# Validation-m3sSAGE/GCN_Recommendation

Hardware: AMD Instinct MI355X
Metric: propagated edges/sec (SpMM) + Recall@20, Amazon-Books 3-layer d=64 (higher is better)
Workload: dtype f32; 1 GPU; C3 full Amazon-Books-2023 shape (10.3M users x 4.4M items x 29.5M interactions); generator=powerlaw, users=10300000, items=4400000, interactions=29500000, nnz=56305746, d=64, layers=3, brands=0, content_dim=0, hub_threshold=128, hub_mode=exact, emu_min_degree=1024, parallelism=single

## Files before the change

gcn_recommendation_amd/csrc/lgcn_engine.hip:

```cpp
#include "lgcn_kernels.h"

#include <string.h>
#include <algorithm>
#include <functional>
#include <new>
#include <vector>

namespace lgcn_detail {
int g_rows_per_group = 0;
int g_unroll = 0;
int g_mean_prefetch = 0;
int g_min_groups = 0;
int g_emu_margin = (128 << 4) | 4;
int g_sample_blocks = 0;
int g_fusion_bwd_blocks = 0;
}

namespace {
__global__ void k_coo_inspect(const int64_t* __restrict__ rows, const int64_t* __restrict__ cols,
                              int64_t nnz, int32_t n_rows, int32_t n_cols, int32_t* flags) {
    const int64_t j = (int64_t)blockIdx.x * blockDim.x + threadIdx.x;
    if (j >= nnz) return;
    const int64_t r = rows[j], c = cols[j];
    int f = 0;
// ... 356 lines not shown

int scale_rows(const lgcn_rows_t& x, int32_t n_rows, int32_t d, float div, float* y, int64_t ldy,
               hipStream_t s, bool sum = false) {
    const bool vec_ok = rows_aligned(x) && al16(y) && (ldy % 4 == 0);
    const Geo g = pick_geo(d, vec_ok);
    ScaleF f{&x, n_rows, g.dW, div, y, ldy, sum, s};
    return dispatch_geo(g, f);
}

struct MeanEmptyF {
    const int32_t* row_ids; int32_t n; const lgcn_rows_t* e0; int32_t dW; float div;
    int32_t inv_bits; float* y; int64_t ldy; hipStream_t s;
    template <typename V, int G, int NV> int operator()() const {
        return launch_mean_empty_t<V, G, NV>(row_ids, n, *e0, dW, div, inv_bits, y, ldy, s);
    }
};

int mean_empty(const int32_t* row_ids, int32_t n, const lgcn_epilogue_t& ep_in, float* y,
               int64_t ldy, int32_t d, hipStream_t s) {
    const lgcn_epilogue_t ep = with_pow2(ep_in);
    const bool vec_ok = rows_aligned(ep.prev0) && al16(y) && (ldy % 4 == 0);
    const Geo g = pick_geo(d, vec_ok);
    MeanEmptyF f{row_ids, n, &ep.prev0, g.dW, ep.div, ep.pad, y, ldy, s};
    return dispatch_geo(g, f);
}

lgcn_rows_t dense_rows(const float* p, int32_t n, int64_t ld) {
    lgcn_rows_t r;
    r.p0 = r.p1 = r.p2 = p;
    r.end0 = r.end1 = n;
    r.ld = ld;
    return r;
}

int valid_geom(int32_t n_rows, int32_t d) {
    if (n_rows < 0 || d < 1 || d > 2048) return LGCN_EINVAL;
    return 0;
}

}

template <typename V>
__global__ __launch_bounds__(256) void k_add_nonzero(const V* __restrict__ src, V* __restrict__ dst,
                                                     int64_t m) {
    for (int64_t i = (int64_t)blockIdx.x * 256 + threadIdx.x; i < m;
         i += (int64_t)gridDim.x * 256) {
// ... 914 lines not shown
        return LGCN_EINVAL;
    for (int i = 0; i < 2 * kSegs; ++i)
        if (int e = check_plan(plans + i)) return e;
    return 0;
}

bool classes_hold(const lgcn_sides_t& sd, const lgcn_hub_plan_t* plans) {
    for (int j = 0; j < 2; ++j) {
        const lgcn_hub_plan_t& p = plans[2 * 3 + j];
        if (p.emu_part_rows[0] > sd.part_rows[0] || p.emu_part_rows[1] > sd.part_rows[1])
            return false;
    }
    return true;
}

struct LayerIO {
    lgcn_rows_t x;
    float xdiv;
    const uint32_t* x_nz;
    float* y;
    lgcn_epilogue_t ep;
};

int seg_layer(const int32_t* rowptr, const lgcn_edge_t* edges, const int32_t* row_ids,
              int32_t lo, int32_t hi, const lgcn_hub_plan_t* plans, int k, int g,
              const LayerIO& io, int32_t d, const lgcn_sched* sc, const Lane& L, Deps* dp,
              int32_t empty_tail = 0) {
    if (empty_tail > 0) {
        hi -= empty_tail;
        if (io.ep.mode == LGCN_EPI_MEAN)
            if (int e = mean_empty(row_ids + hi, empty_tail, io.ep, io.y, d, d, L.main)) return e;
    }
    if (hi <= lo) {
        if (dp && dp->defer && sc)
            for (int i = 0; i < 2; ++i)
                if (int e = record(sc, L.main, &dp->part_done[i])) return e;
        return 0;
    }
    const int h = (k - 1) * kSegs + g;
    lgcn_sched v;
    const lgcn_sched* vp = nullptr;
    if (L.view) {
        v = *L.view;
        v.t0 = sc->timing_sides ? sc->timing_sides[2 * h] : nullptr;
        v.t1 = sc->timing_sides ? sc->timing_sides[2 * h + 1] : nullptr;
        v.trace = sc->trace_sides ? sc->trace_sides + h * 8 : nullptr;
        vp = &v;
    }
    Deps local;
    Deps* dq = dp;
    if (!vp && dp && dp->defer && sc) {
        local = *dp;
        local.defer = false;
        dq = &local;
    }
    if (int e = plan_layer(rowptr + lo, edges, row_ids + lo, hi - lo, plans[2 * g + (k & 1)],
                           io.x, io.xdiv, io.x_nz, io.y, d, d, io.ep, vp, L.main, dq))
        return e;
    if (dq == &local)
        for (int i = 0; i < 2; ++i)
            if (int e = record(sc, L.main, &dp->part_done[i])) return e;
    return 0;
}

int run_sides(const int32_t* rowptr, const lgcn_edge_t* edges, const int32_t* row_ids,
              const lgcn_sides_t& sd, const lgcn_hub_plan_t* plans, int32_t d, int32_t K,
              const std::function<LayerIO(int)>& layer, const lgcn_sched* sched, hipStream_t s,
              const int32_t* empty_tail = nullptr) {
    Lane lanes[2];
    bool l1_aux = false;
    if (sched) sched->pool->next = 0;
    const bool two = make_lanes(sched, s, lanes, l1_aux);
    const bool cap = capture_restricted(s);
    const bool classes = sched && sched->classes && classes_hold(sd, plans) && !cap;
    if (sched) sched->pool->state[3] = classes ? 1 : 0;
    const int32_t lo[kSegs] = {0, sd.class_end[0], sd.class_end[1], sd.split};
    const int32_t hi[kSegs] = {sd.class_end[0], sd.class_end[1], sd.split, 0};
    auto seg_hi = [&](int g, int32_t n) { return g == 3 ? n : hi[g]; };
    const int32_t n = sd.n;
    if (int e = fork_lanes(sched, two, lanes[1], s)) return e;
    constexpr int KM = LGCN_MAX_LAYERS + 2;
    hipEvent_t cls[KM][3] = {}, ab[KM] = {}, rest[KM] = {}, part[KM][2] = {};
    for (int k = 1; k <= K; ++k) {
        const LayerIO io = layer(k);
        const bool mean = io.ep.mode == LGCN_EPI_MEAN;
        {
            const Lane& L = lanes[(k + 1 + K) & 1];
            Deps dp;
            if (classes && k >= 2) {
                dp.part_wait[0] = cls[k - 1][0];
                dp.part_wait[1] = ab[k - 1];
            }
            dp.defer = k < K && sched && !cap;
            if (k == K && mean && sched && sched->lk_normal && two && l1_aux && !cap &&
                sched->n_aux >= 3)
                dp.lk = sched->aux[2];
            if (mean && k >= 2) {
                dp.late[0] = rest[k - 1];
                dp.late_emu[0] = part[k - 1][0];
                dp.late_emu[1] = part[k - 1][1];
            }
            if (int e = seg_layer(rowptr, edges, row_ids, sd.split, n, plans, k, 3, io, d, sched,
                                  L, &dp, empty_tail ? empty_tail[3] : 0))
                return e;
            if (k < K && sched) {
                if (int e = record(sched, L.main, &rest[k])) return e;
                part[k][0] = dp.part_done[0];
                part[k][1] = dp.part_done[1];
            }
        }
        {
            const Lane& L = lanes[(k + K) & 1];
            static const int up[3] = {0, 1, 2}, down[3] = {2, 1, 0};
            const int* order = k == 1 ? up : down;
            for (int t = 0; t < 3; ++t) {
                const int c = order[t];
                if (k >= 2 && (c <= 1 || !classes))
                    if (int e = wait_ev(L.main, part[k - 1][1])) return e;
                if (k >= 2 && (c == 0 || !classes))
                    if (int e = wait_ev(L.main, part[k - 1][0])) return e;
                Deps dp;
                if (mean && k >= 2) dp.late[0] = cls[k - 1][c];
                if (int e = seg_layer(rowptr, edges, row_ids, lo[c], seg_hi(c, n), plans, k, c,
                                      io, d, sched, L, &dp, empty_tail ? empty_tail[c] : 0))
                    return e;
                if (sched)
                    if (int e = record(sched, L.main, &cls[k][c])) return e;
            }
            ab[k] = k == 1 ? cls[k][1] : cls[k][0];
        }
    }
    return join_lanes(sched, two, lanes[1], s);
}
}

extern "C" {

int lgcn_sched_create(void* const* aux_streams, int32_t n_aux, lgcn_sched_t** out) {
    if (!out || n_aux < 1 || n_aux > 7 || !aux_streams) return LGCN_EINVAL;
    for (int i = 0; i < n_aux; ++i)
        if (!aux_streams[i]) return LGCN_EINVAL;
    lgcn_sched* sc = new (std::nothrow) lgcn_sched();
    EventPool* pool = new (std::nothrow) EventPool();
    if (!sc || !pool) {
        delete sc;
        delete pool;
        return LGCN_EINVAL;
// ... 171 lines not shown
int lgcn_propagate_forward_sides(const int32_t* rowptr, const lgcn_edge_t* edges,
                                 const int32_t* row_ids, const lgcn_sides_t* sides,
                                 const lgcn_hub_plan_t* plans, lgcn_rows_t emb, int32_t d,
                                 int32_t K, float* const* layer_bufs_host, float* out,
                                 const lgcn_sched_t* sched, void* stream) {
    return lgcn_propagate_forward_sides_lean(rowptr, edges, row_ids, sides, plans, nullptr, emb, d,
                                             K, layer_bufs_host, out, sched, stream);
}

int lgcn_propagate_forward_sides_lean(const int32_t* rowptr, const lgcn_edge_t* edges,
                                      const int32_t* row_ids, const lgcn_sides_t* sides,
                                      const lgcn_hub_plan_t* plans, const lgcn_lean_t* lean,
                                      lgcn_rows_t emb, int32_t d, int32_t K,
                                      float* const* layer_bufs_host, float* out,
                                      const lgcn_sched_t* sched, void* stream) {
    const int32_t n = sides ? sides->n : -1;
    if (int e = valid_geom(n, d)) return e;
    if (K < 0 || !out) return LGCN_EINVAL;
    if (K > LGCN_MAX_LAYERS) return LGCN_ETOOMANY;
    if (K > 1 && !layer_bufs_host) return LGCN_EINVAL;
    hipStream_t s = S(stream);
    if (K == 0) return scale_rows(emb, n, d, 1.0f, out, d, s, true);
    if (int e = check_sides(rowptr, row_ids, n, sides, plans)) return e;
    auto layer = [&](int k) {
        LayerIO io;
        memset(&io, 0, sizeof(io));
        io.x = (k == 1) ? emb : dense_rows(layer_bufs_host[k - 2], n, d);
        io.xdiv = 1.f;
        if (k < K) {
            io.ep.mode = LGCN_EPI_STORE;
            io.y = layer_bufs_host[k - 1];
        } else {
            io.ep.mode = LGCN_EPI_MEAN;
            io.ep.n_prev = K;
            io.ep.div = (float)(K + 1);
            io.ep.prev0 = emb;
            for (int i = 0; i + 1 < K; ++i) io.ep.prev_dense[i] = layer_bufs_host[i];
            io.ep.ld_prev = d;
            io.y = out;
        }
        return io;
    };
    if (lean) {
        const int32_t b[kSegs + 1] = {0, sides->class_end[0], sides->class_end[1], sides->split, n};
        for (int g = 0; g < kSegs; ++g)
            if (lean->empty_tail[g] < 0 || lean->empty_tail[g] > b[g + 1] - b[g])
                return LGCN_EINVAL;
    }
    return run_sides(rowptr, edges, row_ids, *sides, plans, d, K, layer, sched, s,
                     lean ? lean->empty_tail : nullptr);
}

int lgcn_propagate_backward_sides(const int32_t* rowptr, const lgcn_edge_t* edges,
                                  const int32_t* row_ids, const lgcn_sides_t* sides,
                                  const lgcn_hub_plan_t* plans, lgcn_rows_t grad_out,
                                  const uint32_t* grad_nz, int32_t d, int32_t K, float* work_h,
                                  float* grad_e0, const lgcn_sched_t* sched, void* stream) {
    const int32_t n = sides ? sides->n : -1;
    if (int e = valid_geom(n, d)) return e;
    if (K < 0 || !grad_out.p0 || !grad_e0) return LGCN_EINVAL;
    if (K > LGCN_MAX_LAYERS) return LGCN_ETOOMANY;
    hipStream_t s = S(stream);
    if (K == 0) return scale_rows(grad_out, n, d, 1.0f, grad_e0, d, s);
    if (K > 1 && !work_h) return LGCN_EINVAL;
    if (int e = check_sides(rowptr, row_ids, n, sides, plans)) return e;
    auto out_of = [&](int k) { return ((K - k) % 2 == 0) ? grad_e0 : work_h; };
    auto layer = [&](int k) {
        LayerIO io;
        memset(&io, 0, sizeof(io));
        io.x = k == 1 ? grad_out : dense_rows(out_of(k - 1), n, d);
        io.xdiv = k == 1 ? (float)(K + 1) : 1.f;
        io.x_nz = k == 1 ? grad_nz : nullptr;
        io.y = out_of(k);
// ... 46 lines not shown
```

gcn_recommendation_amd/csrc/lgcn_kernels.h:

```cpp
#pragma once
#include <hip/hip_runtime.h>
#include <hipcub/hipcub.hpp>

#include <stdint.h>
#include <string.h>

#include "lgcn.h"


namespace lgcn_detail {
extern int g_rows_per_group;
extern int g_unroll;
extern int g_mean_prefetch;
extern int g_min_groups;

struct LayerArgs {
    const int32_t* rowptr;
    const lgcn_edge_t* edges;
    const int32_t* row_ids;
    int32_t n_rows, thr;
    const lgcn_hub_item_t* items;
    int32_t n_items;
    float* partials;
    lgcn_rows_t x;
// ... 540 lines not shown
template <typename V, int G, int NV>
__global__ __launch_bounds__(kBlock) void k_mean_empty(const int32_t* __restrict__ row_ids,
                                                       int32_t n_rows, lgcn_rows_t e0, int32_t dW,
                                                       float div, int32_t inv_bits,
                                                       float* __restrict__ y, int64_t ldy) {
    using T = VT<V>;
    constexpr int RPB = kBlock / G;
    const int lane = threadIdx.x & (G - 1);
    const int64_t slot = (int64_t)blockIdx.x * RPB + threadIdx.x / G;
    if (slot >= n_rows) return;
    const int32_t row = row_ids[slot];
    const float* xr = seg_row(e0, row);
#pragma unroll
    for (int q = 0; q < NV; ++q) {
        const int c = lane + q * G;
        if (c < dW)
            store_out<V>(y + (int64_t)row * ldy + c * T::W,
                         div_exact<V>(T::add(load_stream<V>(xr + c * T::W), T::zero()), div,
                                      inv_bits));
    }
}

template <typename V, int G, int NV>
__global__ __launch_bounds__(kBlock) void k_rows_nonzero(lgcn_rows_t x, int32_t n_rows, int32_t dW,
                                                         uint32_t* __restrict__ mask,
                                                         int32_t* __restrict__ count) {
    using T = VT<V>;
    constexpr int RPB = kBlock / G;
    constexpr int ROWS = 256;
    __shared__ uint32_t words[ROWS / 32];
    const int lane = threadIdx.x & (G - 1);
    const int grp = threadIdx.x / G;
    if (threadIdx.x < ROWS / 32) words[threadIdx.x] = 0;
    __syncthreads();
    const int64_t base = (int64_t)blockIdx.x * ROWS;
    for (int i = grp; i < ROWS; i += RPB) {
        const int64_t r = base + i;
        bool nz = false;
        if (r < n_rows) {
            const float* xr = seg_row(x, (int32_t)r);
#pragma unroll
            for (int q = 0; q < NV; ++q) {
                const int c = lane + q * G;
                if (c < dW) {
                    const V v = T::load(xr + c * T::W);
                    if constexpr (T::W == 4) nz |= !(v.x == 0.f && v.y == 0.f && v.z == 0.f && v.w == 0.f);
// ... 166 lines not shown
template <typename V, int G, int NV>
int launch_scale_t(const lgcn_rows_t& x, int32_t n_rows, int32_t dW, float div, float* y,
                   int64_t ldy, bool sum, hipStream_t s) {
    constexpr int RPB = kBlock / G;
    const int64_t grid = ((int64_t)n_rows + RPB - 1) / RPB;
    if (grid == 0) return 0;
    if (sum)
        hipLaunchKernelGGL((k_scale_rows<V, G, NV, true>), dim3((uint32_t)grid), dim3(kBlock), 0,
                           s, x, n_rows, dW, div, y, ldy);
    else
        hipLaunchKernelGGL((k_scale_rows<V, G, NV>), dim3((uint32_t)grid), dim3(kBlock), 0, s, x,
                           n_rows, dW, div, y, ldy);
    return last_err();
}

template <typename V, int G, int NV>
int launch_mean_empty_t(const int32_t* row_ids, int32_t n_rows, const lgcn_rows_t& e0, int32_t dW,
                        float div, int32_t inv_bits, float* y, int64_t ldy, hipStream_t s) {
    constexpr int RPB = kBlock / G;
    const int64_t grid = ((int64_t)n_rows + RPB - 1) / RPB;
    if (grid == 0) return 0;
    hipLaunchKernelGGL((k_mean_empty<V, G, NV>), dim3((uint32_t)grid), dim3(kBlock), 0, s, row_ids,
                       n_rows, e0, dW, div, inv_bits, y, ldy);
    return last_err();
}

template <typename F>
int dispatch_geo(const Geo& g, const F& f) {
#define LGCN_CASE(VT_, G_, NV_) \
    if (g.G == G_ && g.NV == NV_) return f.template operator()<VT_, G_, NV_>();
    if (g.vec) {
        LGCN_CASE(float4, 4, 1)
        LGCN_CASE(float4, 8, 1)
        LGCN_CASE(float4, 16, 1)
        LGCN_CASE(float4, 32, 1)
        LGCN_CASE(float4, 64, 1)
        LGCN_CASE(float4, 64, 2)
        LGCN_CASE(float4, 64, 4)
        LGCN_CASE(float4, 64, 8)
    } else {
        LGCN_CASE(float, 4, 1)
        LGCN_CASE(float, 8, 1)
        LGCN_CASE(float, 16, 1)
        LGCN_CASE(float, 32, 1)
        LGCN_CASE(float, 64, 1)
        LGCN_CASE(float, 64, 2)
// ... 28 lines not shown
```

gcn_recommendation_amd/engine.py:

```python
import ctypes
import os
import threading

import numpy as np
import torch

_PKG = os.path.dirname(os.path.abspath(__file__))
LIB_PATH = os.path.join(_PKG, "liblgcn_engine.so")

LGCN_EPI_STORE, LGCN_EPI_MEAN, LGCN_EPI_ADD = 0, 1, 2
LGCN_SCATTER_STORE, LGCN_SCATTER_ADD = 0, 1
LGCN_MAX_LAYERS = 16
COO_ROWS_UNSORTED, COO_OUT_OF_RANGE, COO_COLS_UNSORTED = 1, 2, 4
INT32_MAX = 2 ** 31 - 1
TUNE_ROWS_PER_GROUP, TUNE_UNROLL, TUNE_MEAN_PREFETCH, TUNE_MIN_GROUPS = 1, 2, 3, 4
TUNE_EMU_MARGIN = 6
TUNE_SAMPLE_BLOCKS = 7
TUNE_FUSION_BWD_BLOCKS = 8
FUSION_BWD_CHUNK = 2048
SCHED_SLOTS0, SCHED_SLOTS1, SCHED_CHAIN, SCHED_TIMING_START, SCHED_TIMING_END, SCHED_TRACE = \
    1, 2, 3, 4, 5, 6
SCHED_TRACE_SIDES, SCHED_TIMING_SIDES = 7, 8
SCHED_CLASSES = 16
SCHED_LK_NORMAL = 17
# ... 60 lines not shown
                ("addend", RowsT), ("addend_nz", ctypes.c_void_p)]


class PlanT(ctypes.Structure):
    _fields_ = [("items", ctypes.c_void_p), ("rows", ctypes.c_void_p), ("partials", ctypes.c_void_p),
                ("emu_blocks", ctypes.c_void_p), ("emu_rows", ctypes.c_void_p),
                ("emu_rel", ctypes.c_void_p), ("emu_meta", ctypes.c_void_p),
                ("emu_stage", ctypes.c_void_p),
                ("threshold", ctypes.c_int32), ("n_items", ctypes.c_int32),
                ("n_rows", ctypes.c_int32), ("n_pre", ctypes.c_int32),
                ("n_emu_blocks", ctypes.c_int32), ("n_emu_rows", ctypes.c_int32),
                ("emu_part_rows", ctypes.c_int32 * 2), ("emu_part_blocks", ctypes.c_int32 * 2),
                ("emu_scratch_blocks", ctypes.c_int32), ("emu_live", ctypes.c_void_p),
                ("emu_part_max_blocks", ctypes.c_int32 * 2), ("emu_out", ctypes.c_void_p)]


class SidesT(ctypes.Structure):
    _fields_ = [("n", ctypes.c_int32), ("split", ctypes.c_int32), ("class_end", ctypes.c_int32 * 2),
                ("part_rows", ctypes.c_int32 * 2)]


class LeanT(ctypes.Structure):
    _fields_ = [("empty_tail", ctypes.c_int32 * 4)]


class AdamTensorT(ctypes.Structure):
    _fields_ = [("p", ctypes.c_void_p), ("g", ctypes.c_void_p), ("m", ctypes.c_void_p),
                ("v", ctypes.c_void_p), ("n", ctypes.c_int64), ("step_size", ctypes.c_double),
                ("bc2_sqrt", ctypes.c_double)]


class AdamHyperT(ctypes.Structure):
    _fields_ = [("lerp_w", ctypes.c_double), ("beta2", ctypes.c_double),
                ("one_minus_beta2", ctypes.c_double), ("eps", ctypes.c_double),
                ("weight_decay", ctypes.c_double)]


class LgcnError(RuntimeError):
    pass


_lib = None
_lib_lock = threading.Lock()

_P, _I32, _I64 = ctypes.c_void_p, ctypes.c_int32, ctypes.c_int64
ABI = [
# ... 75 lines not shown
    ("lgcn_live_scratch_bytes", ctypes.c_size_t, [_I32, _I32]),
    ("lgcn_live_rows", ctypes.c_int, [_P, _P, _I32, _P, _I32, RowsT, ctypes.c_float, _P, _P, _I64,
                                      _I32, ctypes.POINTER(EpilogueT), _I32, _I32, _P, _P]),
    ("lgcn_live_flags", ctypes.c_void_p, [_P, _I32, _I32]),
    ("lgcn_chain_rows", ctypes.c_int, [_P, _P, _P, _I32, RowsT, ctypes.c_float, _P, _I64, _I32,
                                       ctypes.POINTER(EpilogueT), _P]),
    ("lgcn_sched_create", ctypes.c_int, [_P, _I32, ctypes.POINTER(ctypes.c_void_p)]),
    ("lgcn_sched_destroy", ctypes.c_int, [_P]),
    ("lgcn_sched_set", ctypes.c_int, [_P, _I32, _I64]),
    ("lgcn_sched_state", ctypes.c_int64, [_P, _I32]),
    ("lgcn_layer", ctypes.c_int, [_P, _P, _P, _I32, ctypes.POINTER(PlanT), RowsT, ctypes.c_float, _P,
                                  _P, _I64, _I32, ctypes.POINTER(EpilogueT), _P, _P]),
    ("lgcn_propagate_forward", ctypes.c_int, [_P, _P, _P, _I32, ctypes.POINTER(PlanT), RowsT, _I32,
                                              _I32, _P, _P, _P, _P, _P]),
    ("lgcn_propagate_backward", ctypes.c_int, [_P, _P, _P, _I32, ctypes.POINTER(PlanT), RowsT, _P,
                                               _I32, _I32, _P, _P, _P, _P]),
    ("lgcn_propagate_forward_sides", ctypes.c_int, [_P, _P, _P, ctypes.POINTER(SidesT),
                                                    ctypes.POINTER(PlanT), RowsT, _I32, _I32, _P,
                                                    _P, _P, _P]),
    ("lgcn_propagate_forward_sides_lean", ctypes.c_int, [_P, _P, _P, ctypes.POINTER(SidesT),
                                                         ctypes.POINTER(PlanT),
                                                         ctypes.POINTER(LeanT), RowsT, _I32, _I32,
                                                         _P, _P, _P, _P]),
    ("lgcn_propagate_backward_sides", ctypes.c_int, [_P, _P, _P, ctypes.POINTER(SidesT),
                                                     ctypes.POINTER(PlanT), RowsT, _P, _I32, _I32,
                                                     _P, _P, _P, _P]),
    ("lgcn_adam_step", ctypes.c_int, [ctypes.POINTER(AdamTensorT), _I32,
                                      ctypes.POINTER(AdamHyperT), _P]),
    ("lgcn_adam_chunks", ctypes.c_int64, [_I64]),
]


def load_library(path=None):
    global _lib
    with _lib_lock:
        if _lib is not None:
            return _lib
        p = path or os.environ.get("LGCN_LIB") or LIB_PATH
        if not os.path.exists(p):
            raise LgcnError(f"liblgcn_engine.so not found at {p}: run `python -c \"import "
                            f"__graft_entry__ as g; g.build()\"` (hipcc --offload-arch=gfx950)")
        lib = ctypes.CDLL(p)
        for name, res, args in ABI:
            fn = getattr(lib, name)
            fn.restype = res
            fn.argtypes = args
# ... 272 lines not shown
        rows[big, 2] = ng
    n_slots = n_chunks + pre.shape[0]
    table = np.concatenate([pre, rows]).astype(np.int32)
    return HubPlan(threshold, mode, chunk, torch.from_numpy(items).to(device),
                   torch.from_numpy(table).to(device), n_slots, hub.size, pre.shape[0])


class Graph:

    def __init__(self, n_rows, n_cols, rowptr, edges, nnz, device, row_ids=None):
        self.n_rows, self.n_cols, self.nnz = n_rows, n_cols, nnz
        self.rowptr, self.edges, self.device = rowptr, edges, device
        self.row_ids = row_ids
        self.transpose = None
        self.symmetric = None
        self.sides = None
        self.split = None
        self.class_end = None
        self.class_parts = (0, 0)
        self._plans = {}
        self._rowptr_host = None
        self._row_ids_host = None
        self._lean = None

    def rowptr_host(self):
        if self._rowptr_host is None:
            self._rowptr_host = self.rowptr.cpu().numpy()
        return self._rowptr_host

    def row_ids_host(self):
        if self.row_ids is None:
            return None
        if self._row_ids_host is None:
            self._row_ids_host = self.row_ids.cpu().numpy()
        return self._row_ids_host

    def hubs(self, threshold, chunk=None, mode=None, emu_min=None):
        mode = mode or hub_mode_from_env()
        if mode not in HUB_MODES:
            raise LgcnError(f"unknown hub mode {mode!r}")
        emu_min = emu_min_degree_from_env(self.nnz) if emu_min is None else emu_min
        chunk = chunk or hub_chunk_for(self.nnz)
        key = (threshold, mode) + ((chunk, DEFAULT_HUB_PRE_GROUP) if mode == "chunk" else (emu_min,))
        if key not in self._plans:
            self._plans[key] = plan_hubs(self.rowptr_host(), threshold, chunk, self.device,
                                         self.row_ids_host(), mode=mode, emu_min=emu_min)
# ... 16 lines not shown
            raise LgcnError("side_hubs needs a side-ordered graph (graph_from_coo(adj, sides=...))")
        mode = mode or hub_mode_from_env()
        if mode not in HUB_MODES:
            raise LgcnError(f"unknown hub mode {mode!r}")
        emu_min = emu_min_degree_from_env(self.nnz) if emu_min is None else emu_min
        chunk = chunk or hub_chunk_for(self.nnz)
        key = ("sides", threshold, mode) + \
            ((chunk, DEFAULT_HUB_PRE_GROUP) if mode == "chunk" else (emu_min,))
        if key not in self._plans:
            rp, ids = self.rowptr_host(), self.row_ids_host()
            self._plans[key] = [
                plan_hubs(rp[a:b + 1], threshold, chunk, self.device, ids[a:b], mode=mode,
                          emu_min=emu_min)
                for a, b in self.segments()]
        return self._plans[key]

    def lean(self):
        if self.split is None:
            raise LgcnError("lean needs a side-ordered graph (graph_from_coo(adj, sides=...))")
        if self._lean is None:
            self._lean = lean_plan(self.rowptr, self.edges, self.row_ids, self.split,
                                   self.segments())
        return self._lean

    @property
    def n_empty(self):
        return self.lean().n_empty

    @property
    def n_derived(self):
        return self.lean().n_derived

    def degrees(self):
        deg = np.diff(self.rowptr_host().astype(np.int64))
        ids = self.row_ids_host()
        if ids is None:
            return deg
        out = np.empty_like(deg)
        out[ids] = deg
        return out


def _bitmask(flags):
    n = flags.numel()
    pad = torch.zeros(((n + 31) // 32) * 32, dtype=torch.int64, device=flags.device)
    pad[:n] = flags
# ... 28 lines not shown
    deg = torch.zeros(n, dtype=torch.int64, device=dev)
    deg[ids] = deg_slot
    named = torch.zeros(n, dtype=torch.bool, device=dev)
    named[col] = True
    empty = (deg == 0) & ~named
    one_slot = deg_slot == 1
    first = rec[rowptr[:-1].long()[one_slot]]
    p = torch.full((n,), -1, dtype=torch.int64, device=dev)
    w = torch.zeros(n, dtype=torch.int64, device=dev)
    p[ids[one_slot]] = first & 0xffffffff
    w[ids[one_slot]] = first >> 32
    side0 = torch.zeros(n, dtype=torch.bool, device=dev)
    side0[ids[:split]] = True
    other = torch.zeros(n, dtype=torch.bool, device=dev)
    other[col[(row != p[col]) | (bits != w[col])]] = True
    derived = (deg == 1) & side0 & ~other
    tails = []
    for a, b in segments:
        e = empty[ids[a:b]]
        live = torch.nonzero(~e)
        tails.append(int(b - a - (int(live[-1]) + 1 if live.numel() else 0)))
    return LeanPlan(_bitmask(empty), _bitmask(derived), int(empty.sum()), int(derived.sum()),
                    tails)


def slot_key_enabled(g):
    return g.n_rows == g.n_cols and os.environ.get("LGCN_SLOT_KEY", "1") != "0"


def order_by_degree(lib, g, stream, sides=None):
    n, nnz, dev = g.n_rows, g.nnz, g.device
    lo, hi = sides if sides is not None else (0, 0)
    i32 = dict(dtype=torch.int32, device=dev)
    deg_tmp, deg_sorted, iota = (torch.empty(max(n, 1), **i32) for _ in range(3))
    row_ids = torch.empty(max(n, 1), **i32)
    rowptr = torch.empty(n + 1, **i32)
    edges = torch.empty(max(nnz, 1), dtype=torch.int64, device=dev)
    keys = (torch.empty(max(n, 1), dtype=torch.int64, device=dev) for _ in range(2)) \
        if slot_key_enabled(g) else (None, None)
    key_tmp, key_sorted = keys
    nbytes = ctypes.c_size_t(0)
    args = (_ptr(g.rowptr), _ptr(g.edges), n, nnz, lo, hi, _ptr(deg_tmp), _ptr(deg_sorted),
            _ptr(iota),
            _ptr(row_ids), _ptr(rowptr), _ptr(edges),
            _ptr(key_tmp) if key_tmp is not None else None,
            _ptr(key_sorted) if key_sorted is not None else None)
# ... 449 lines not shown
    segs = [g for g, (a, b) in enumerate(graph.segments()) if b > a]
    if ev.timing is not None and side_timing is not None:
        side_timing.append({(k, g): (ev.timing[((k - 1) * N_SEGS + g) * 2],
                                     ev.timing[((k - 1) * N_SEGS + g) * 2 + 1])
                            for k in range(1, K + 1) for g in segs})
    if ev.trace is not None and side_trace is not None:
        side_trace.append({(k, g): list(zip(TRACE_PHASES,
                                            ev.trace[((k - 1) * N_SEGS + g) * 8:
                                                     ((k - 1) * N_SEGS + g + 1) * 8]))
                           for k in range(1, K + 1) for g in segs})


def _check_depth(K):
    if K > LGCN_MAX_LAYERS or K < 0:
        raise LgcnError(f"n_layers={K} unsupported (0..{LGCN_MAX_LAYERS})")


def alloc_layers(n, d, count, device):
    return [torch.empty((n, d), dtype=torch.float32, device=device) for _ in range(count)]


def propagate_forward(graph, segments, K, hub_threshold=None, layer_events=None,
                      return_layers=False, hub_mode=None, emu_min=None, kernel_events=None,
                      lean=None):
    if hub_threshold is None:
        hub_threshold = hub_threshold_from_env()
    d = segments[0].shape[1]
    n = sum(int(t.shape[0]) for t in segments)
    if n != graph.n_rows:
        raise LgcnError(f"embedding rows {n} != adjacency size {graph.n_rows}")
    _check_emb(segments, d, graph.device)
    _check_depth(K)
    lib = load_library()
    dev = graph.device
    with torch.cuda.device(dev):
        stream = _stream(dev)
        e0 = rows_desc(segments, d)
        out = torch.empty((n, d), dtype=torch.float32, device=dev)
        if K == 0:
            _check(lib.lgcn_propagate_forward(None, None, None, n, None, e0, d, 0, None,
                                              _ptr(out), None, None, stream),
                   "lgcn_propagate_forward")
            return (out, []) if return_layers else out
        layers = alloc_layers(n, d, K - 1, dev)
        if use_sides(graph, layer_events, kernel_events):
            if lean is None:
                lean = not return_layers
            lp = graph.lean().struct() if lean else None
            plans, _ = _side_plans(graph, d, hub_threshold, hub_mode, emu_min,
                                   _aligned16(segments))
            sc = sched_for(dev)
            ev = _SideEvents(sc, K, side_timing is not None, side_trace is not None)
            bufs = (ctypes.c_void_p * max(K - 1, 1))(*[t.data_ptr() for t in layers])
            sides = graph.sides_struct()
            try:
                _check(lib.lgcn_propagate_forward_sides_lean(
                    _ptr(graph.rowptr), _ptr(graph.edges), _ptr(graph.row_ids),
                    ctypes.byref(sides), plans, ctypes.byref(lp) if lp is not None else None,
                    e0, d, K, bufs, _ptr(out),
                    sc.handle if sc is not None else None, stream),
                    "lgcn_propagate_forward_sides_lean")
            finally:
                ev.clear()
            _note_schedule(sc, graph)
            _collect_sides(ev, K, graph)
            return (out, layers) if return_layers else out
        hp = graph.hubs(hub_threshold, mode=hub_mode, emu_min=emu_min)
        for k in range(1, K + 1):
            xs = segments if k == 1 else [layers[k - 2]]
            if k < K:
                y, ep = layers[k - 1], _epilogue(LGCN_EPI_STORE)
            else:
                y = out
                ep = _epilogue(LGCN_EPI_MEAN, prev0=e0, prev_dense=layers, ld_prev=d,
                               div=float(K + 1))
            if layer_events is not None:
                layer_events[k - 1][0].record()
            spmm_layer(graph, xs, y, d, ep, hub_threshold, hp, stream,
                       kernel_events=None if kernel_events is None else kernel_events[k - 1])
            if layer_events is not None:
                layer_events[k - 1][1].record()
        return (out, layers) if return_layers else out


# ... 241 lines not shown
```

include/lgcn.h:

```cpp
#ifndef LGCN_H_
#define LGCN_H_

#include <stdint.h>
#include <stddef.h>

#ifdef __cplusplus
extern "C" {
#endif

#define LGCN_ABI_VERSION 14

#define LGCN_EINVAL      (-1)
#define LGCN_EALIGN      (-2)
#define LGCN_ETOOMANY    (-3)

#define LGCN_MAX_LAYERS 16

#define LGCN_COO_ROWS_UNSORTED   1
#define LGCN_COO_OUT_OF_RANGE    2
#define LGCN_COO_COLS_UNSORTED   4

#define LGCN_EPI_STORE 0
#define LGCN_EPI_MEAN  1
#define LGCN_EPI_ADD   2
// ... 240 lines not shown
                            const uint32_t* grad_nz, int32_t d, int32_t K, float* work_h,
                            float* grad_e0, const lgcn_sched_t* sched, void* stream);

typedef struct {
    int32_t n;
    int32_t split;
    int32_t class_end[2];
    int32_t part_rows[2];
} lgcn_sides_t;
int lgcn_propagate_forward_sides(const int32_t* rowptr, const lgcn_edge_t* edges,
                                 const int32_t* row_ids, const lgcn_sides_t* sides,
                                 const lgcn_hub_plan_t* plans, lgcn_rows_t emb, int32_t d,
                                 int32_t K, float* const* layer_bufs_host, float* out,
                                 const lgcn_sched_t* sched, void* stream);
typedef struct {
    int32_t empty_tail[4];
} lgcn_lean_t;
int lgcn_propagate_forward_sides_lean(const int32_t* rowptr, const lgcn_edge_t* edges,
                                      const int32_t* row_ids, const lgcn_sides_t* sides,
                                      const lgcn_hub_plan_t* plans, const lgcn_lean_t* lean,
                                      lgcn_rows_t emb, int32_t d, int32_t K,
                                      float* const* layer_bufs_host, float* out,
                                      const lgcn_sched_t* sched, void* stream);
int lgcn_propagate_backward_sides(const int32_t* rowptr, const lgcn_edge_t* edges,
                                  const int32_t* row_ids, const lgcn_sides_t* sides,
                                  const lgcn_hub_plan_t* plans, lgcn_rows_t grad_out,
                                  const uint32_t* grad_nz, int32_t d, int32_t K, float* work_h,
                                  float* grad_e0, const lgcn_sched_t* sched, void* stream);

int lgcn_bpr_loss(const float* u, int64_t ldu, const float* p, int64_t ldp, const float* n,
                  int64_t ldn, const float* u0, int64_t ldu0, const float* p0, int64_t ldp0,
                  const float* n0, int64_t ldn0, int32_t B, int32_t d, float lambda, float* terms,
                  float* loss, float* grads, void* stream);

int lgcn_bpr_loss_indexed(const float* fu, int64_t ld_fu, const float* fi, int64_t ld_fi,
                          const float* u0, int64_t ld_u0, const float* i0, int64_t ld_i0,
                          int64_t n_users, int64_t n_items, const int64_t* users,
                          const int64_t* pos, const int64_t* neg, int32_t B, int32_t d,
                          float lambda, float* terms, float* loss, float* grads, void* stream);

int lgcn_bpr_keys(const int64_t* users, const int64_t* pos, const int64_t* neg, int32_t B,
                  int64_t n_users, int64_t n_items, int64_t* keys, void* stream);

#define LGCN_SCATTER_STORE 0
#define LGCN_SCATTER_ADD   1
int lgcn_rows_scatter(const int32_t* keys_sorted, const int32_t* perm, int32_t n, const float* src,
// ... 92 lines not shown
```

Baseline: 14.85 billion edges/s.

## Deduplicate degree-one rows sharing a neighbor and read representative rows

Adds a shared-row plan that finds degree-one rows whose single edge targets the same column. Those rows are grouped behind a representative, and edges in later layers are remapped to the representative's id. The duplicate rows then skip the intermediate layers and get their final mean from a dedicated kernel that reads the representative's layer values, optionally on an auxiliary stream overlapping the main SpMM. This trades extra preprocessing, cloned edge arrays and more stream synchronisation for less intermediate-layer work. Whether the equivalence holds depends on the lean plan's 'derived' row semantics.

```diff
diff --git a/gcn_recommendation_amd/csrc/lgcn_engine.hip b/gcn_recommendation_amd/csrc/lgcn_engine.hip
--- a/gcn_recommendation_amd/csrc/lgcn_engine.hip
+++ b/gcn_recommendation_amd/csrc/lgcn_engine.hip
@@ -402,6 +402,26 @@
     const bool vec_ok = rows_aligned(ep.prev0) && al16(y) && (ldy % 4 == 0);
     const Geo g = pick_geo(d, vec_ok);
     MeanEmptyF f{row_ids, n, &ep.prev0, g.dW, ep.div, ep.pad, y, ldy, s};
+    return dispatch_geo(g, f);
+}
+
+struct MeanSharedF {
+    const int32_t* rowptr; const lgcn_edge_t* edges; const int32_t* row_ids; const int32_t* rep;
+    int32_t n; const lgcn_rows_t* x; int32_t dW; const lgcn_epilogue_t* ep; float* y; int64_t ldy;
+    hipStream_t s;
+    template <typename V, int G, int NV> int operator()() const {
+        return launch_mean_shared_t<V, G, NV>(rowptr, edges, row_ids, rep, n, *x, dW, *ep, y, ldy,
+                                              s);
+    }
+};
+
+int mean_shared(const int32_t* rowptr, const lgcn_edge_t* edges, const int32_t* row_ids,
+                const int32_t* rep, int32_t n, const lgcn_rows_t& x, const lgcn_epilogue_t& ep_in,
+                float* y, int64_t ldy, int32_t d, hipStream_t s) {
+    const lgcn_epilogue_t ep = with_pow2(ep_in);
+    const bool vec_ok = rows_aligned(x) && al16(y) && (ldy % 4 == 0) && epi_aligned(ep);
+    const Geo g = pick_geo(d, vec_ok);
+    MeanSharedF f{rowptr, edges, row_ids, rep, n, &x, g.dW, &ep, y, ldy, s};
     return dispatch_geo(g, f);
 }
 
@@ -1362,20 +1382,58 @@
     lgcn_epilogue_t ep;
 };
 
+LayerIO forward_io(int k, int32_t K, const lgcn_rows_t& emb, float* const* layer_bufs_host,
+                   float* out, int32_t n, int32_t d) {
+    LayerIO io;
+    memset(&io, 0, sizeof(io));
+    io.x = (k == 1) ? emb : dense_rows(layer_bufs_host[k - 2], n, d);
+    io.xdiv = 1.f;
+    if (k < K) {
+        io.ep.mode = LGCN_EPI_STORE;
+        io.y = layer_bufs_host[k - 1];
+    } else {
+        io.ep.mode = LGCN_EPI_MEAN;
+        io.ep.n_prev = K;
+        io.ep.div = (float)(K + 1);
+        io.ep.prev0 = emb;
+        for (int i = 0; i + 1 < K; ++i) io.ep.prev_dense[i] = layer_bufs_host[i];
+        io.ep.ld_prev = d;
+        io.y = out;
+    }
+    return io;
+}
+
 int seg_layer(const int32_t* rowptr, const lgcn_edge_t* edges, const int32_t* row_ids,
               int32_t lo, int32_t hi, const lgcn_hub_plan_t* plans, int k, int g,
               const LayerIO& io, int32_t d, const lgcn_sched* sc, const Lane& L, Deps* dp,
-              int32_t empty_tail = 0) {
+              int32_t empty_tail = 0, int32_t shared_tail = 0, const int32_t* rep = nullptr) {
     if (empty_tail > 0) {
         hi -= empty_tail;
         if (io.ep.mode == LGCN_EPI_MEAN)
             if (int e = mean_empty(row_ids + hi, empty_tail, io.ep, io.y, d, d, L.main)) return e;
     }
+    hi -= shared_tail;
+    const bool has_shared = shared_tail > 0 && io.ep.mode == LGCN_EPI_MEAN;
+    auto shared_mean = [&](hipStream_t st) -> int {
+        if (!has_shared) return 0;
+        return mean_shared(rowptr + hi, edges, row_ids + hi, rep, shared_tail, io.x, io.ep, io.y,
+                           d, d, st);
+    };
+    hipStream_t side = nullptr;
+    if (has_shared && hi > lo && L.view && L.view->n_aux > 0 &&
+        !capture_restricted(L.main)) {
+        side = L.view->aux[L.view->n_aux > 1 ? 1 : 0];
+        if (int e = link(sc, L.main, side)) return e;
+        if (int e = wait_late(side, dp)) return e;
+        if (int e = shared_mean(side)) return e;
+    }
     if (hi <= lo) {
         if (dp && dp->defer && sc)
             for (int i = 0; i < 2; ++i)
                 if (int e = record(sc, L.main, &dp->part_done[i])) return e;
-        return 0;
+        if (has_shared)
+            if (int e = wait_late(L.main, dp)) return e;
+        return shared_mean(L.main);
     }
     const int h = (k - 1) * kSegs + g;
     lgcn_sched v;
@@ -1400,13 +1458,18 @@
     if (dq == &local)
         for (int i = 0; i < 2; ++i)
             if (int e = record(sc, L.main, &dp->part_done[i])) return e;
-    return 0;
+    if (side) return link(sc, side, L.main);
+    return shared_mean(L.main);
 }
 
 int run_sides(const int32_t* rowptr, const lgcn_edge_t* edges, const int32_t* row_ids,
               const lgcn_sides_t& sd, const lgcn_hub_plan_t* plans, int32_t d, int32_t K,
               const std::function<LayerIO(int)>& layer, const lgcn_sched* sched, hipStream_t s,
-              const int32_t* empty_tail = nullptr) {
+              const int32_t* empty_tail = nullptr, const lgcn_shared_t* sh = nullptr) {
+    const lgcn_edge_t* edges_ln = sh ? sh->edges_ln : edges;
+    int32_t rep_off[kSegs] = {0, 0, 0, 0};
+    if (sh)
+        for (int g = 1; g < kSegs; ++g) rep_off[g] = rep_off[g - 1] + sh->shared_tail[g - 1];
     Lane lanes[2];
     bool l1_aux = false;
     if (sched) sched->pool->next = 0;
@@ -1440,8 +1503,8 @@
                 dp.late_emu[0] = part[k - 1][0];
                 dp.late_emu[1] = part[k - 1][1];
             }
-            if (int e = seg_layer(rowptr, edges, row_ids, sd.split, n, plans, k, 3, io, d, sched,
-                                  L, &dp, empty_tail ? empty_tail[3] : 0))
+            if (int e = seg_layer(rowptr, k >= 2 ? edges_ln : edges, row_ids, sd.split, n, plans,
+                                  k, 3, io, d, sched, L, &dp, empty_tail ? empty_tail[3] : 0))
                 return e;
             if (k < K && sched) {
                 if (int e = record(sched, L.main, &rest[k])) return e;
@@ -1462,7 +1525,9 @@
                 Deps dp;
                 if (mean && k >= 2) dp.late[0] = cls[k - 1][c];
                 if (int e = seg_layer(rowptr, edges, row_ids, lo[c], seg_hi(c, n), plans, k, c,
-                                      io, d, sched, L, &dp, empty_tail ? empty_tail[c] : 0))
+                                      io, d, sched, L, &dp, empty_tail ? empty_tail[c] : 0,
+                                      sh ? sh->shared_tail[c] : 0,
+                                      sh ? sh->rep + rep_off[c] : nullptr))
                     return e;
                 if (sched)
                     if (int e = record(sched, L.main, &cls[k][c])) return e;
@@ -1680,25 +1745,7 @@
     hipStream_t s = S(stream);
     if (K == 0) return scale_rows(emb, n, d, 1.0f, out, d, s, true);
     if (int e = check_sides(rowptr, row_ids, n, sides, plans)) return e;
-    auto layer = [&](int k) {
-        LayerIO io;
-        memset(&io, 0, sizeof(io));
-        io.x = (k == 1) ? emb : dense_rows(layer_bufs_host[k - 2], n, d);
-        io.xdiv = 1.f;
-        if (k < K) {
-            io.ep.mode = LGCN_EPI_STORE;
-            io.y = layer_bufs_host[k - 1];
-        } else {
-            io.ep.mode = LGCN_EPI_MEAN;
-            io.ep.n_prev = K;
-            io.ep.div = (float)(K + 1);
-            io.ep.prev0 = emb;
-            for (int i = 0; i + 1 < K; ++i) io.ep.prev_dense[i] = layer_bufs_host[i];
-            io.ep.ld_prev = d;
-            io.y = out;
-        }
-        return io;
-    };
+    auto layer = [&](int k) { return forward_io(k, K, emb, layer_bufs_host, out, n, d); };
     if (lean) {
         const int32_t b[kSegs + 1] = {0, sides->class_end[0], sides->class_end[1], sides->split, n};
         for (int g = 0; g < kSegs; ++g)
@@ -1707,6 +1754,35 @@
     }
     return run_sides(rowptr, edges, row_ids, *sides, plans, d, K, layer, sched, s,
                      lean ? lean->empty_tail : nullptr);
+}
+
+int lgcn_propagate_forward_sides_shared(const int32_t* rowptr, const lgcn_sides_t* sides,
+                                        const lgcn_hub_plan_t* plans, const lgcn_shared_t* sh,
+                                        lgcn_rows_t emb, int32_t d, int32_t K,
+                                        float* const* layer_bufs_host, float* out,
+                                        const lgcn_sched_t* sched, void* stream) {
+    const int32_t n = sides ? sides->n : -1;
+    if (int e = valid_geom(n, d)) return e;
+    if (K < 0 || !out || !sh) return LGCN_EINVAL;
+    if (K > LGCN_MAX_LAYERS) return LGCN_ETOOMANY;
+    if (K > 1 && !layer_bufs_host) return LGCN_EINVAL;
+    hipStream_t s = S(stream);
+    if (K == 0) return scale_rows(emb, n, d, 1.0f, out, d, s, true);
+    if (int e = check_sides(rowptr, sh->row_ids, n, sides, plans)) return e;
+    const int32_t b[kSegs + 1] = {0, sides->class_end[0], sides->class_end[1], sides->split, n};
+    bool any = false;
+    for (int g = 0; g < kSegs; ++g) {
+        const int32_t et = sh->empty_tail[g], st = sh->shared_tail[g];
+        if (et < 0 || st < 0 || (int64_t)et + st > b[g + 1] - b[g]) return LGCN_EINVAL;
+        any = any || st > 0;
+    }
+    if (sh->shared_tail[3] != 0) return LGCN_EINVAL;
+    if ((sh->shared_tail[0] > 0) + (sh->shared_tail[1] > 0) + (sh->shared_tail[2] > 0) > 1)
+        return LGCN_EINVAL;
+    if (any && (!sh->row_ids || !sh->edges_l1 || !sh->edges_ln || !sh->rep)) return LGCN_EINVAL;
+    auto layer = [&](int k) { return forward_io(k, K, emb, layer_bufs_host, out, n, d); };
+    return run_sides(rowptr, sh->edges_l1, sh->row_ids, *sides, plans, d, K, layer, sched, s,
+                     sh->empty_tail, K >= 2 && any ? sh : nullptr);
 }
 
 int lgcn_propagate_backward_sides(const int32_t* rowptr, const lgcn_edge_t* edges,
diff --git a/gcn_recommendation_amd/csrc/lgcn_kernels.h b/gcn_recommendation_amd/csrc/lgcn_kernels.h
--- a/gcn_recommendation_amd/csrc/lgcn_kernels.h
+++ b/gcn_recommendation_amd/csrc/lgcn_kernels.h
@@ -586,6 +586,38 @@
 }
 
 template <typename V, int G, int NV>
+__global__ __launch_bounds__(kBlock) void k_mean_shared(const int32_t* __restrict__ rowptr,
+                                                        const lgcn_edge_t* __restrict__ edges,
+                                                        const int32_t* __restrict__ row_ids,
+                                                        const int32_t* __restrict__ rep,
+                                                        int32_t n_rows, lgcn_rows_t x, int32_t dW,
+                                                        lgcn_epilogue_t ep, float* __restrict__ y,
+                                                        int64_t ldy) {
+    using T = VT<V>;
+    constexpr int RPB = kBlock / G;
+    const int lane = threadIdx.x & (G - 1);
+    const int64_t slot = (int64_t)blockIdx.x * RPB + threadIdx.x / G;
+    if (slot >= n_rows) return;
+    const int32_t row = row_ids[slot];
+    const int32_t r = rep[slot];
+    const int2 e = load_edge(edges + rowptr[slot]);
+    const float w = __int_as_float(e.y);
+    const float* xp = seg_row(x, e.x);
+    const float* e0 = seg_row(ep.prev0, row);
+#pragma unroll
+    for (int q = 0; q < NV; ++q) {
+        const int c = lane + q * G;
+        if (c >= dW) continue;
+        const V acc = T::fma(w, T::load(xp + c * T::W), T::zero());
+        V s = T::add(T::zero(), load_stream<V>(e0 + c * T::W));
+        for (int i = 0; i + 1 < ep.n_prev; ++i)
+            s = T::add(s, T::load(ep.prev_dense[i] + (int64_t)r * ep.ld_prev + c * T::W));
+        s = T::add(s, acc);
+        store_out<V>(y + (int64_t)row * ldy + c * T::W, div_exact<V>(s, ep.div, ep.pad));
+    }
+}
+
+template <typename V, int G, int NV>
 __global__ __launch_bounds__(kBlock) void k_rows_nonzero(lgcn_rows_t x, int32_t n_rows, int32_t dW,
                                                          uint32_t* __restrict__ mask,
                                                          int32_t* __restrict__ count) {
@@ -798,6 +830,18 @@
     if (grid == 0) return 0;
     hipLaunchKernelGGL((k_mean_empty<V, G, NV>), dim3((uint32_t)grid), dim3(kBlock), 0, s, row_ids,
                        n_rows, e0, dW, div, inv_bits, y, ldy);
+    return last_err();
+}
+
+template <typename V, int G, int NV>
+int launch_mean_shared_t(const int32_t* rowptr, const lgcn_edge_t* edges, const int32_t* row_ids,
+                         const int32_t* rep, int32_t n_rows, const lgcn_rows_t& x, int32_t dW,
+                         const lgcn_epilogue_t& ep, float* y, int64_t ldy, hipStream_t s) {
+    constexpr int RPB = kBlock / G;
+    const int64_t grid = ((int64_t)n_rows + RPB - 1) / RPB;
+    if (grid == 0) return 0;
+    hipLaunchKernelGGL((k_mean_shared<V, G, NV>), dim3((uint32_t)grid), dim3(kBlock), 0, s, rowptr,
+                       edges, row_ids, rep, n_rows, x, dW, ep, y, ldy);
     return last_err();
 }
 
diff --git a/gcn_recommendation_amd/engine.py b/gcn_recommendation_amd/engine.py
--- a/gcn_recommendation_amd/engine.py
+++ b/gcn_recommendation_amd/engine.py
@@ -106,6 +106,12 @@
 
 class LeanT(ctypes.Structure):
     _fields_ = [("empty_tail", ctypes.c_int32 * 4)]
+
+
+class SharedT(ctypes.Structure):
+    _fields_ = [("empty_tail", ctypes.c_int32 * 4), ("shared_tail", ctypes.c_int32 * 4),
+                ("row_ids", ctypes.c_void_p), ("edges_l1", ctypes.c_void_p),
+                ("edges_ln", ctypes.c_void_p), ("rep", ctypes.c_void_p)]
 
 
 class AdamTensorT(ctypes.Structure):
@@ -227,6 +233,10 @@
                                                          ctypes.POINTER(PlanT),
                                                          ctypes.POINTER(LeanT), RowsT, _I32, _I32,
                                                          _P, _P, _P, _P]),
+    ("lgcn_propagate_forward_sides_shared", ctypes.c_int, [_P, ctypes.POINTER(SidesT),
+                                                           ctypes.POINTER(PlanT),
+                                                           ctypes.POINTER(SharedT), RowsT, _I32,
+                                                           _I32, _P, _P, _P, _P]),
     ("lgcn_propagate_backward_sides", ctypes.c_int, [_P, _P, _P, ctypes.POINTER(SidesT),
                                                      ctypes.POINTER(PlanT), RowsT, _P, _I32, _I32,
                                                      _P, _P, _P, _P]),
@@ -545,6 +555,7 @@
         self._rowptr_host = None
         self._row_ids_host = None
         self._lean = None
+        self._shared = None
 
     def rowptr_host(self):
         if self._rowptr_host is None:
@@ -607,6 +618,20 @@
             self._lean = lean_plan(self.rowptr, self.edges, self.row_ids, self.split,
                                    self.segments())
         return self._lean
+
+    def shared(self):
+        if self._shared is None:
+            self._shared = shared_plan(self.rowptr, self.edges, self.row_ids, self.split,
+                                       self.segments(), self.lean())
+        return self._shared
+
+    @property
+    def n_shared(self):
+        return self.shared().n_shared
+
+    @property
+    def n_groups(self):
+        return self.shared().n_groups
 
     @property
     def n_empty(self):
@@ -681,6 +706,93 @@
         tails.append(int(b - a - (int(live[-1]) + 1 if live.numel() else 0)))
     return LeanPlan(_bitmask(empty), _bitmask(derived), int(empty.sum()), int(derived.sum()),
                     tails)
+
+
+def _unmask(words, n):
+    sh = torch.arange(32, dtype=torch.int64, device=words.device)
+    return (((words.long().unsqueeze(1) >> sh) & 1).reshape(-1)[:n]).bool()
+
+
+class SharedPlan:
+
+    def __init__(self, row_ids_s, edges_l1, edges_ln, rep, empty_tail, shared_tail, tail_slots,
+                 n_shared, n_groups):
+        self.row_ids_s, self.edges_l1, self.edges_ln, self.rep = row_ids_s, edges_l1, edges_ln, rep
+        self.empty_tail, self.shared_tail = tuple(empty_tail), tuple(shared_tail)
+        self.tail_slots = tuple(tail_slots)
+        self.n_shared, self.n_groups = n_shared, n_groups
+
+    def shared_rows(self):
+        return torch.cat([self.row_ids_s[a:b] for a, b in self.tail_slots]).long()
+
+    def struct(self):
+        st = SharedT()
+        for g in range(N_SEGS):
+            st.empty_tail[g], st.shared_tail[g] = self.empty_tail[g], self.shared_tail[g]
+        st.row_ids, st.edges_l1 = self.row_ids_s.data_ptr(), self.edges_l1.data_ptr()
+        st.edges_ln, st.rep = self.edges_ln.data_ptr(), self.rep.data_ptr()
+        return st
+
+
+def shared_plan(rowptr, edges, row_ids, split, segments, lean):
+    dev = rowptr.device
+    n = rowptr.numel() - 1
+    nnz = int(rowptr[-1])
+    ids = row_ids.long()
+    i64 = dict(dtype=torch.int64, device=dev)
+    tails, tail_slots = [0] * N_SEGS, [(b, b) for _, b in segments]
+    none = SharedPlan(row_ids, edges, edges, torch.zeros(0, dtype=torch.int32, device=dev),
+                      lean.empty_tail, tails, tail_slots, 0, 0)
+    side0 = [g for g, (a, b) in enumerate(segments[:3]) if b > a]
+    if len(side0) != 1 or nnz == 0:
+        return none
+    g = side0[0]
+    a, b = segments[g]
+    deg = (rowptr[a + 1:b + 1] - rowptr[a:b]).long()
+    one = torch.nonzero(deg == 1).flatten()
+    if one.numel() == 0:
+        return none
+    s0, s1 = a + int(one[0]), a + int(one[-1]) + 1
+    if s1 - s0 != one.numel() or s1 != b - lean.empty_tail[g]:
+        return none
+    m = s1 - s0
+    pos = rowptr[s0:s1].long()
+    rec = edges[pos]
+    ci = torch.nonzero(_unmask(lean.derived, n)[ids[s0:s1]]).flatten()
+    if ci.numel() == 0:
+        return none
+    keys, perm = torch.sort(rec[ci], stable=True)
+    first = torch.ones_like(keys, dtype=torch.bool)
+    first[1:] = keys[1:] != keys[:-1]
+    at = torch.arange(keys.numel(), **i64)
+    start = torch.cummax(torch.where(first, at, torch.zeros_like(at)), 0).values
+    rep_slot = torch.full((m,), -1, **i64)
+    rep_slot[ci[perm[~first]]] = ci[perm[start]][~first]
+    is_shared = rep_slot >= 0
+    sh = torch.nonzero(is_shared).flatten()
+    n_groups, n_shared = int(first.sum()), int(sh.numel())
+    if n_shared == 0:
+        none.n_groups = n_groups
+        return none
+    order = torch.cat([torch.nonzero(~is_shared).flatten(), sh])
+    row_ids_s = row_ids.clone()
+    row_ids_s[s0:s1] = row_ids[s0:s1][order]
+    edges_l1 = edges.clone()
+    edges_l1[pos] = rec[order]
+    rep_rows = ids[s0 + rep_slot[sh]]
+    new_id = torch.arange(n, **i64)
+    new_id[ids[s0 + sh]] = rep_rows
+    edges_ln = edges_l1.clone()
+    r = edges_l1[:nnz]
+    edges_ln[:nnz] = ((r >> 32) << 32) | new_id[r & 0xffffffff]
+    tails[g] = n_shared
+    tail_slots[g] = (s1 - n_shared, s1)
+    return SharedPlan(row_ids_s, edges_l1, edges_ln, rep_rows.to(torch.int32), lean.empty_tail,
+                      tails, tail_slots, n_shared, n_groups)
+
+
+def share_enabled():
+    return os.environ.get("LGCN_SHARE", "1") != "0"
 
 
 def slot_key_enabled(g):
@@ -1176,7 +1288,7 @@
 
 def propagate_forward(graph, segments, K, hub_threshold=None, layer_events=None,
                       return_layers=False, hub_mode=None, emu_min=None, kernel_events=None,
-                      lean=None):
+                      lean=None, share=None):
     if hub_threshold is None:
         hub_threshold = hub_threshold_from_env()
     d = segments[0].shape[1]
@@ -1198,9 +1310,16 @@
             return (out, []) if return_layers else out
         layers = alloc_layers(n, d, K - 1, dev)
         if use_sides(graph, layer_events, kernel_events):
+            if share is None:
+                share = lean is not False and not return_layers and share_enabled()
             if lean is None:
-                lean = not return_layers
+                lean = share or not return_layers
+            if share and not lean:
+                raise LgcnError("share=True needs lean: the shared rows sit before the empty tail")
             lp = graph.lean().struct() if lean else None
+            sp = graph.shared() if share and K >= 2 and hub_threshold >= 1 else None
+            if sp is not None and sp.n_shared == 0:
+                sp = None
             plans, _ = _side_plans(graph, d, hub_threshold, hub_mode, emu_min,
                                    _aligned16(segments))
             sc = sched_for(dev)
@@ -1208,12 +1327,19 @@
             bufs = (ctypes.c_void_p * max(K - 1, 1))(*[t.data_ptr() for t in layers])
             sides = graph.sides_struct()
             try:
-                _check(lib.lgcn_propagate_forward_sides_lean(
-                    _ptr(graph.rowptr), _ptr(graph.edges), _ptr(graph.row_ids),
-                    ctypes.byref(sides), plans, ctypes.byref(lp) if lp is not None else None,
-                    e0, d, K, bufs, _ptr(out),
-                    sc.handle if sc is not None else None, stream),
-                    "lgcn_propagate_forward_sides_lean")
+                if sp is not None:
+                    st = sp.struct()
+                    _check(lib.lgcn_propagate_forward_sides_shared(
+                        _ptr(graph.rowptr), ctypes.byref(sides), plans, ctypes.byref(st), e0, d, K,
+                        bufs, _ptr(out), sc.handle if sc is not None else None, stream),
+                        "lgcn_propagate_forward_sides_shared")
+                else:
+                    _check(lib.lgcn_propagate_forward_sides_lean(
+                        _ptr(graph.rowptr), _ptr(graph.edges), _ptr(graph.row_ids),
+                        ctypes.byref(sides), plans, ctypes.byref(lp) if lp is not None else None,
+                        e0, d, K, bufs, _ptr(out),
+                        sc.handle if sc is not None else None, stream),
+                        "lgcn_propagate_forward_sides_lean")
             finally:
                 ev.clear()
             _note_schedule(sc, graph)
diff --git a/include/lgcn.h b/include/lgcn.h
--- a/include/lgcn.h
+++ b/include/lgcn.h
@@ -286,6 +286,18 @@
                                       lgcn_rows_t emb, int32_t d, int32_t K,
                                       float* const* layer_bufs_host, float* out,
                                       const lgcn_sched_t* sched, void* stream);
+typedef struct {
+    int32_t empty_tail[4], shared_tail[4];
+    const int32_t* row_ids;
+    const lgcn_edge_t* edges_l1;
+    const lgcn_edge_t* edges_ln;
+    const int32_t* rep;
+} lgcn_shared_t;
+int lgcn_propagate_forward_sides_shared(const int32_t* rowptr, const lgcn_sides_t* sides,
+                                        const lgcn_hub_plan_t* plans, const lgcn_shared_t* shared,
+                                        lgcn_rows_t emb, int32_t d, int32_t K,
+                                        float* const* layer_bufs_host, float* out,
+                                        const lgcn_sched_t* sched, void* stream);
 int lgcn_propagate_backward_sides(const int32_t* rowptr, const lgcn_edge_t* edges,
                                   const int32_t* row_ids, const lgcn_sides_t* sides,
                                   const lgcn_hub_plan_t* plans, lgcn_rows_t grad_out,
```

Result: faster. 15.44 billion edges/s, median of 6 (+4.0%).
